# oso95/Agentainer-lab

Measured on AMD Instinct MI355X. Metric: concurrent_agent_chat_req_per_s, higher is better.
Workload: dtype bf16; 1 GPU; model=llama3-8b, agents_per_gpu=64, agents=64, global_batch=64, prompt_len=256, gen_len=57, seq_len=313, parallelism=dp1

## Files before the change

### agentainer_amd/ops/csrc/decode_attn.hip

```cpp

#include <torch/extension.h>
#include <ATen/hip/HIPContext.h>
#include <cfloat>
#include "common.h"

namespace {

constexpr int CHUNK = 64;
constexpr int SPLITS = 8;
constexpr int PART_STRIDE = 132;

template <int RATIO, int D, typename CT>
__global__ __launch_bounds__(64) void decode_partial_kernel(
    float* __restrict__ part,
    const short* __restrict__ q,
    const CT* __restrict__ k_cache,
    const CT* __restrict__ v_cache,
    const int* __restrict__ page_table,
    const int* __restrict__ seq_lens,
    float scale, int n_q, int n_kv, int PS, int max_pages, long q_ts) {
  constexpr bool FP8 = sizeof(CT) == 1;
  const int b = blockIdx.x;
  const int g = blockIdx.y;
  const int split = blockIdx.z;
  const int lane = threadIdx.x;
  const int len = seq_lens[b];
  constexpr int D8 = D / 8;

  float* my_part = part +
      ((((long)b * gridDim.y + g) * SPLITS + split) * RATIO) * PART_STRIDE;

  const int n_chunks = (len + CHUNK - 1) / CHUNK;
  const int cpw = (n_chunks + SPLITS - 1) / SPLITS;
  const int c0 = split * cpw;
  const int c1 = min(c0 + cpw, n_chunks);
  if (len <= 0 || c0 >= c1) {
    for (int h = 0; h < RATIO; ++h) {
      float* pp = my_part + h * PART_STRIDE;
      pp[2 * lane] = 0.f;
      pp[2 * lane + 1] = 0.f;
      if (lane == 0) { pp[128] = -FLT_MAX; pp[129] = 0.f; }
    }
    return;
  }

  __shared__ float p_lds[RATIO][CHUNK];
  const int qh0 = g * RATIO;
  const int ds = lane / 16;
  const int t16 = lane % 16;
  typedef __bf16 bf2 __attribute__((ext_vector_type(2)));
  __shared__ short q_lds[RATIO][D];
#pragma unroll
  for (int h = 0; h < RATIO; ++h) {
    const short* qp = q + (long)b * q_ts + (long)(qh0 + h) * D;
#pragma unroll
    for (int r = 0; r < D / WAVE; ++r)
      q_lds[h][r * WAVE + lane] = qp[r * WAVE + lane];
  }
  __builtin_amdgcn_s_waitcnt(0);

  constexpr int Q8S = D + 8;
  __shared__ unsigned char q8_lds[16 * Q8S];
  __shared__ float qsc_lds[16];
  if constexpr (sizeof(CT) == 1) {
#pragma unroll
    for (int h = 0; h < 16; ++h) {
      float sc = 0.f;
      if (h < RATIO) {
        float mx = fmaxf(fabsf(bits2f(q_lds[h][2 * lane])),
                         fabsf(bits2f(q_lds[h][2 * lane + 1])));
        mx = wave_max(mx);
        sc = fmaxf(mx, 1e-8f) / 448.f;
        const float inv = 1.f / sc;
        q8_lds[h * Q8S + 2 * lane] =
            f2fp8(bits2f(q_lds[h][2 * lane]) * inv);
        q8_lds[h * Q8S + 2 * lane + 1] =
            f2fp8(bits2f(q_lds[h][2 * lane + 1]) * inv);
      } else {
        q8_lds[h * Q8S + 2 * lane] = 0;
        q8_lds[h * Q8S + 2 * lane + 1] = 0;
      }
      if (lane == 0) qsc_lds[h] = sc;
    }
    __builtin_amdgcn_s_waitcnt(0);
  }

  const int pv_tg = lane / 16;
  const int pv_dg = lane % 16;
  float m[RATIO], l[RATIO];
  float o[RATIO][8];
#pragma unroll
  for (int h = 0; h < RATIO; ++h) {
    m[h] = -FLT_MAX; l[h] = 0.f;
#pragma unroll
    for (int j = 0; j < 8; ++j) o[h][j] = 0.f;
  }
  const int* pt = page_table + (long)b * max_pages;

  for (int c = c0; c < c1; ++c) {
    if constexpr (FP8) {
      __shared__ float cm_b[16], cs_b[16], mn_b[16];
      const int myh = lane % 16;
      float sv[16];
#pragma unroll
      for (int gt = 0; gt < 4; ++gt) {
        const int tok = c * CHUNK + gt * 16 + (lane % 16);
        const int tok_c = min(tok, len - 1);
        const long page = pt[tok_c / PS];
        const CT* kp = k_cache +
            ((long)page * n_kv + g) * D8 * PS * 8 + (tok_c % PS) * 8;
        f32x4 acc = {0.f, 0.f, 0.f, 0.f};
#pragma unroll
        for (int dc = 0; dc < 4; ++dc) {
          long a, bq;
          __builtin_memcpy(&a, kp + (long)(dc * 4 + lane / 16) * PS * 8, 8);
          __builtin_memcpy(&bq, &q8_lds[myh * Q8S + dc * 32 + (lane / 16) * 8],
                           8);
          acc = __builtin_amdgcn_mfma_f32_16x16x32_fp8_fp8(a, bq, acc, 0, 0, 0);
        }
#pragma unroll
        for (int r = 0; r < 4; ++r) sv[gt * 4 + r] = acc[r];
      }
      const float qs = qsc_lds[myh] * scale;
      float cmax = -FLT_MAX;
#pragma unroll
      for (int gt = 0; gt < 4; ++gt)
#pragma unroll
        for (int r = 0; r < 4; ++r) {
          const int tok = c * CHUNK + gt * 16 + (lane / 16) * 4 + r;
          const float v = (tok < len) ? sv[gt * 4 + r] * qs : -FLT_MAX;
          sv[gt * 4 + r] = v;
          cmax = fmaxf(cmax, v);
        }
      cmax = fmaxf(cmax, __shfl_xor(cmax, 16, WAVE));
      cmax = fmaxf(cmax, __shfl_xor(cmax, 32, WAVE));
      if (lane < 16) cm_b[myh] = cmax;
      __builtin_amdgcn_s_waitcnt(0);
      float alpha_s[RATIO];
#pragma unroll
      for (int h = 0; h < RATIO; ++h) {
        const float mn = fmaxf(m[h], cm_b[h]);
        alpha_s[h] = (m[h] == -FLT_MAX) ? 0.f : __expf(m[h] - mn);
#pragma unroll
        for (int j = 0; j < 8; ++j) o[h][j] *= alpha_s[h];
        m[h] = mn;
        if (lane == 0) mn_b[h] = mn;
      }
      __builtin_amdgcn_s_waitcnt(0);
      const float mn_my = mn_b[myh];
      float csum = 0.f;
#pragma unroll
      for (int gt = 0; gt < 4; ++gt)
#pragma unroll
        for (int r = 0; r < 4; ++r) {
          const int t = gt * 16 + (lane / 16) * 4 + r;
          const float pv = (sv[gt * 4 + r] == -FLT_MAX)
                               ? 0.f
                               : __expf(sv[gt * 4 + r] - mn_my);
          if (myh < RATIO) p_lds[myh][t] = pv;
          csum += pv;
        }
      csum += __shfl_xor(csum, 16, WAVE);
      csum += __shfl_xor(csum, 32, WAVE);
      if (lane < 16) cs_b[myh] = csum;
      __builtin_amdgcn_s_waitcnt(0);
#pragma unroll
      for (int h = 0; h < RATIO; ++h) l[h] = l[h] * alpha_s[h] + cs_b[h];
    } else {
    float s[4][RATIO];
#pragma unroll
    for (int sub = 0; sub < 4; ++sub) {
      const int tok = c * CHUNK + sub * 16 + t16;
      float acc[RATIO];
#pragma unroll
      for (int h = 0; h < RATIO; ++h) acc[h] = 0.f;
      if (tok < len) {
        const long page = pt[tok / PS];
        const CT* kp = k_cache +
            ((long)page * n_kv + g) * D8 * PS * 8 + (tok % PS) * 8;
        {
          bf16x8 kv[4];
#pragma unroll
          for (int r = 0; r < 4; ++r)
            kv[r] = *reinterpret_cast<const bf16x8*>(
                kp + (long)(r * 4 + ds) * PS * 8);
#pragma unroll
          for (int r = 0; r < 4; ++r) {
            const bf2* kp2 = reinterpret_cast<const bf2*>(&kv[r]);
#pragma unroll
            for (int h = 0; h < RATIO; ++h) {
              const bf16x8 qv8 = *reinterpret_cast<const bf16x8*>(
                  &q_lds[h][(r * 4 + ds) * 8]);
              const bf2* qp2 = reinterpret_cast<const bf2*>(&qv8);
#pragma unroll
              for (int j = 0; j < 4; ++j)
                acc[h] = __builtin_amdgcn_fdot2_f32_bf16(kp2[j], qp2[j],
                                                         acc[h], false);
            }
          }
        }
      }
#pragma unroll
      for (int h = 0; h < RATIO; ++h) {
        acc[h] += __shfl_xor(acc[h], 16, WAVE);
        acc[h] += __shfl_xor(acc[h], 32, WAVE);
        s[sub][h] = (tok < len) ? acc[h] * scale : -FLT_MAX;
      }
    }
#pragma unroll
    for (int h = 0; h < RATIO; ++h) {
      float cm = fmaxf(fmaxf(s[0][h], s[1][h]), fmaxf(s[2][h], s[3][h]));
      cm = wave_max(cm);
      const float mn = fmaxf(m[h], cm);
      float psum = 0.f;
#pragma unroll
      for (int sub = 0; sub < 4; ++sub) {
        const float p = (s[sub][h] == -FLT_MAX) ? 0.f : __expf(s[sub][h] - mn);
        if (ds == 0) {
          p_lds[h][sub * 16 + t16] = p;
          psum += p;
        }
      }
      const float csum = wave_sum(psum);
      const float alpha = (m[h] == -FLT_MAX) ? 0.f : __expf(m[h] - mn);
      l[h] = l[h] * alpha + csum;
#pragma unroll
      for (int j = 0; j < 8; ++j) o[h][j] *= alpha;
      m[h] = mn;
    }
    __builtin_amdgcn_s_waitcnt(0);
    }

    const int base_tok = c * CHUNK;
#pragma unroll 4
    for (int u = 0; u < 16; ++u) {
      const int t = u * 4 + pv_tg;
      const int gt = base_tok + t;
      const int gt_c = min(gt, len - 1);
      const long page = pt[gt_c / PS];
      const CT* vp = v_cache +
          (((long)page * n_kv + g) * PS + gt_c % PS) * D + pv_dg * 8;
      float vf[8];
      if constexpr (FP8) {
        const u8x8 vv = *reinterpret_cast<const u8x8*>(vp);
        fp8x8_to_f32(vv, vf);
      } else {
        const bf16x8 vv = *reinterpret_cast<const bf16x8*>(vp);
#pragma unroll
        for (int j = 0; j < 8; ++j) vf[j] = bits2f(vv[j]);
      }
#pragma unroll
      for (int h = 0; h < RATIO; ++h) {
        const float pw = p_lds[h][t];
#pragma unroll
        for (int j = 0; j < 8; ++j)
          o[h][j] = fmaf(pw, vf[j], o[h][j]);
      }
    }
  }

#pragma unroll
  for (int h = 0; h < RATIO; ++h) {
    float* pp = my_part + h * PART_STRIDE;
#pragma unroll
    for (int j = 0; j < 8; ++j) {
      float v = o[h][j];
      v += __shfl_xor(v, 16, WAVE);
      v += __shfl_xor(v, 32, WAVE);
      if (pv_tg == 0) pp[pv_dg * 8 + j] = v;
    }
    if (lane == 0) { pp[128] = m[h]; pp[129] = l[h]; }
  }
}

template <int D>
__global__ __launch_bounds__(64) void decode_combine_kernel(
    short* __restrict__ out,
    const float* __restrict__ part,
    const int* __restrict__ seq_lens, int n_q, int n_kv) {
  const int b = blockIdx.x;
  const int qh = blockIdx.y;
  const int lane = threadIdx.x;
  if (seq_lens[b] <= 0) return;
  const int ratio = n_q / n_kv;
  const int g = qh / ratio;
  const int h = qh % ratio;
  const float* pp = part +
      ((((long)b * n_kv + g) * SPLITS) * ratio + h) * PART_STRIDE;
  const long step = (long)ratio * PART_STRIDE;

  float M = -FLT_MAX;
#pragma unroll
  for (int s = 0; s < SPLITS; ++s) M = fmaxf(M, pp[s * step + 128]);
  float L = 0.f, O0 = 0.f, O1 = 0.f;
#pragma unroll
  for (int s = 0; s < SPLITS; ++s) {
    const float ms = pp[s * step + 128];
    if (ms == -FLT_MAX) continue;
    const float w = __expf(ms - M);
    L += w * pp[s * step + 129];
    O0 = fmaf(w, pp[s * step + 2 * lane], O0);
    O1 = fmaf(w, pp[s * step + 2 * lane + 1], O1);
  }
  const float inv = (L > 0.f) ? 1.0f / L : 0.f;
  short* op = out + ((long)b * n_q + qh) * D + 2 * lane;
  op[0] = f2bits(O0 * inv);
  op[1] = f2bits(O1 * inv);
}

}

void paged_decode_attention_ws(torch::Tensor out, torch::Tensor q,
                               torch::Tensor k_cache, torch::Tensor v_cache,
                               torch::Tensor page_table, torch::Tensor seq_lens,
                               torch::Tensor workspace, double scale) {
  TORCH_CHECK(out.is_contiguous());
  TORCH_CHECK(q.scalar_type() == at::kBFloat16);
  TORCH_CHECK(page_table.scalar_type() == at::kInt &&
              seq_lens.scalar_type() == at::kInt);
  TORCH_CHECK(workspace.scalar_type() == at::kFloat);
  TORCH_CHECK(q.stride(2) == 1 && q.stride(1) == q.size(2));
  const int B = q.size(0), n_q = q.size(1), D = q.size(2);
  const int n_kv = k_cache.size(1), PS = k_cache.size(3);
  const int max_pages = page_table.size(1);
  const int ratio = n_q / n_kv;
  TORCH_CHECK(D == 128, "decode attention: head_dim 128 only");
  TORCH_CHECK(n_q % n_kv == 0);
  TORCH_CHECK(workspace.numel() >=
              (long)B * n_kv * SPLITS * ratio * PART_STRIDE,
              "decode workspace too small");
  if (B == 0) return;
  auto stream = at::hip::getCurrentHIPStream();
  dim3 grid1(B, n_kv, SPLITS);
  const bool fp8 = k_cache.scalar_type() == at::kFloat8_e4m3fn;
#define LAUNCH_RATIO_CT(R, CT)                                                 \
  hipLaunchKernelGGL((decode_partial_kernel<R, 128, CT>), grid1, dim3(64), 0,  \
                     stream, workspace.data_ptr<float>(),                      \
                     (const short*)q.data_ptr(),                               \
                     (const CT*)k_cache.data_ptr(),                            \
                     (const CT*)v_cache.data_ptr(),                            \
                     page_table.data_ptr<int>(), seq_lens.data_ptr<int>(),     \
                     (float)scale, n_q, n_kv, PS, max_pages,                    \
                     (long)q.stride(0))
#define LAUNCH_RATIO(R)                                                        \
  do {                                                                         \
    if (fp8) LAUNCH_RATIO_CT(R, unsigned char);                                \
    else LAUNCH_RATIO_CT(R, short);                                            \
  } while (0)
  switch (ratio) {
    case 1: LAUNCH_RATIO(1); break;
    case 2: LAUNCH_RATIO(2); break;
    case 4: LAUNCH_RATIO(4); break;
    case 8: LAUNCH_RATIO(8); break;
    default:
      TORCH_CHECK(false, "decode attention: GQA ratio must be 1/2/4/8, got ",
                  ratio);
  }
#undef LAUNCH_RATIO
#undef LAUNCH_RATIO_CT
  hipLaunchKernelGGL((decode_combine_kernel<128>), dim3(B, n_q), dim3(64), 0,
                     stream, (short*)out.data_ptr(),
                     workspace.data_ptr<float>(), seq_lens.data_ptr<int>(),
                     n_q, n_kv);
}

long decode_attention_workspace_size(long B, long n_q, long n_kv) {
  return B * n_kv * SPLITS * (n_q / n_kv) * PART_STRIDE;
}

void paged_decode_attention(torch::Tensor out, torch::Tensor q,
                            torch::Tensor k_cache, torch::Tensor v_cache,
                            torch::Tensor page_table, torch::Tensor seq_lens,
                            double scale) {
  const int B = q.size(0), n_q = q.size(1);
  const int n_kv = k_cache.size(1);
  auto ws = torch::empty(
      {decode_attention_workspace_size(B, n_q, n_kv)},
      torch::TensorOptions().dtype(torch::kFloat).device(q.device()));
  paged_decode_attention_ws(out, q, k_cache, v_cache, page_table, seq_lens,
                            ws, scale);
}
```

Baseline: 126.0 req/s.

## Fuse split-K decode attention and combine into one multi-wave block kernel

Replaces the two-kernel split-K decode attention (partial kernel over a SPLITS grid dimension, then a combine kernel through a global workspace) with a single kernel. Each block runs SPLITS waves, the partial results are merged in LDS, and the workspace round trip and second launch go away. For power-of-two page sizes it also adds a FAST path: page ids are prefetched one chunk ahead with readfirstlane and shift/mask addressing, K loads for a whole chunk are batched, and V uses a sliding prefetch window. Full waitcnt(0) calls are relaxed to LDS-only waits. The trade-offs are fewer blocks (B*n_kv instead of B*n_kv*SPLITS), higher register pressure from the buffered loads, and removal of the workspace-based API entry points that other code may still call.

```diff
diff --git a/agentainer_amd/ops/csrc/decode_attn.hip b/agentainer_amd/ops/csrc/decode_attn.hip
--- a/agentainer_amd/ops/csrc/decode_attn.hip
+++ b/agentainer_amd/ops/csrc/decode_attn.hip
@@ -10,61 +10,68 @@
 constexpr int SPLITS = 8;
 constexpr int PART_STRIDE = 132;
 
-template <int RATIO, int D, typename CT>
-__global__ __launch_bounds__(64) void decode_partial_kernel(
-    float* __restrict__ part,
+template <int D>
+__device__ __forceinline__ void merge_partials(short* __restrict__ op,
+                                               const float* pp, int step,
+                                               int lane) {
+  float M = -FLT_MAX;
+#pragma unroll
+  for (int s = 0; s < SPLITS; ++s) M = fmaxf(M, pp[s * step + 128]);
+  float L = 0.f, O0 = 0.f, O1 = 0.f;
+#pragma unroll
+  for (int s = 0; s < SPLITS; ++s) {
+    const float ms = pp[s * step + 128];
+    if (ms == -FLT_MAX) continue;
+    const float w = __expf(ms - M);
+    L += w * pp[s * step + 129];
+    O0 = fmaf(w, pp[s * step + 2 * lane], O0);
+    O1 = fmaf(w, pp[s * step + 2 * lane + 1], O1);
+  }
+  const float inv = (L > 0.f) ? 1.0f / L : 0.f;
+  op[0] = f2bits(O0 * inv);
+  op[1] = f2bits(O1 * inv);
+}
+
+template <int RATIO, int D, typename CT, bool FAST>
+__global__ __launch_bounds__(SPLITS * WAVE) void decode_attn_kernel(
+    short* __restrict__ out,
     const short* __restrict__ q,
     const CT* __restrict__ k_cache,
     const CT* __restrict__ v_cache,
     const int* __restrict__ page_table,
     const int* __restrict__ seq_lens,
-    float scale, int n_q, int n_kv, int PS, int max_pages, long q_ts) {
+    float scale, int n_q, int n_kv, int PS, int ps_shift, int max_pages,
+    long q_ts) {
   constexpr bool FP8 = sizeof(CT) == 1;
+  constexpr int D8 = D / 8;
+  constexpr int VWIN = 8;
   const int b = blockIdx.x;
   const int g = blockIdx.y;
-  const int split = blockIdx.z;
-  const int lane = threadIdx.x;
+  const int split = __builtin_amdgcn_readfirstlane(threadIdx.x / WAVE);
+  const int lane = threadIdx.x % WAVE;
   const int len = seq_lens[b];
-  constexpr int D8 = D / 8;
-
-  float* my_part = part +
-      ((((long)b * gridDim.y + g) * SPLITS + split) * RATIO) * PART_STRIDE;
-
-  const int n_chunks = (len + CHUNK - 1) / CHUNK;
-  const int cpw = (n_chunks + SPLITS - 1) / SPLITS;
-  const int c0 = split * cpw;
-  const int c1 = min(c0 + cpw, n_chunks);
-  if (len <= 0 || c0 >= c1) {
-    for (int h = 0; h < RATIO; ++h) {
-      float* pp = my_part + h * PART_STRIDE;
-      pp[2 * lane] = 0.f;
-      pp[2 * lane + 1] = 0.f;
-      if (lane == 0) { pp[128] = -FLT_MAX; pp[129] = 0.f; }
-    }
-    return;
-  }
-
-  __shared__ float p_lds[RATIO][CHUNK];
+  if (len <= 0) return;
+
+  __shared__ float part_lds[SPLITS][RATIO][PART_STRIDE];
+  __shared__ float p_all[SPLITS][RATIO][CHUNK];
+  float (*p_lds)[CHUNK] = p_all[split];
   const int qh0 = g * RATIO;
   const int ds = lane / 16;
   const int t16 = lane % 16;
   typedef __bf16 bf2 __attribute__((ext_vector_type(2)));
   __shared__ short q_lds[RATIO][D];
-#pragma unroll
-  for (int h = 0; h < RATIO; ++h) {
-    const short* qp = q + (long)b * q_ts + (long)(qh0 + h) * D;
-#pragma unroll
-    for (int r = 0; r < D / WAVE; ++r)
-      q_lds[h][r * WAVE + lane] = qp[r * WAVE + lane];
-  }
-  __builtin_amdgcn_s_waitcnt(0);
+  for (int i = threadIdx.x; i < RATIO * D; i += SPLITS * WAVE)
+    q_lds[i / D][i % D] = q[(long)b * q_ts + (long)(qh0 + i / D) * D + i % D];
+  __syncthreads();
 
   constexpr int Q8S = D + 8;
-  __shared__ unsigned char q8_lds[16 * Q8S];
+  __shared__ unsigned char q8_lds[FP8 ? 16 * Q8S : 1];
   __shared__ float qsc_lds[16];
-  if constexpr (sizeof(CT) == 1) {
-#pragma unroll
-    for (int h = 0; h < 16; ++h) {
+  __shared__ float cm_all[SPLITS][16], cs_all[SPLITS][16], mn_all[SPLITS][16];
+  if constexpr (FP8) {
+#pragma unroll
+    for (int hh = 0; hh < 16 / SPLITS; ++hh) {
+      const int h = split + hh * SPLITS;
       float sc = 0.f;
       if (h < RATIO) {
         float mx = fmaxf(fabsf(bits2f(q_lds[h][2 * lane])),
@@ -82,7 +89,7 @@
       }
       if (lane == 0) qsc_lds[h] = sc;
     }
-    __builtin_amdgcn_s_waitcnt(0);
+    __syncthreads();
   }
 
   const int pv_tg = lane / 16;
@@ -96,30 +103,99 @@
     for (int j = 0; j < 8; ++j) o[h][j] = 0.f;
   }
   const int* pt = page_table + (long)b * max_pages;
+  const int psm = PS - 1;
+
+  const int n_chunks = (len + CHUNK - 1) / CHUNK;
+  const int cpw = (n_chunks + SPLITS - 1) / SPLITS;
+  const int c0 = split * cpw;
+  const int c1 = min(c0 + cpw, n_chunks);
+
+  int pid_n[4] = {0, 0, 0, 0};
+  if constexpr (FAST) {
+    if (c0 < c1) {
+#pragma unroll
+      for (int j = 0; j < 4; ++j)
+        pid_n[j] = __builtin_amdgcn_readfirstlane(
+            pt[min(c0 * CHUNK + j * 16, len - 1) >> ps_shift]);
+    }
+  }
+
+  using VT = typename std::conditional<FP8, u8x8, bf16x8>::type;
 
   for (int c = c0; c < c1; ++c) {
+    int pid[4];
+#pragma unroll
+    for (int j = 0; j < 4; ++j) pid[j] = pid_n[j];
+    if constexpr (FAST) {
+#pragma unroll
+      for (int j = 0; j < 4; ++j)
+        pid_n[j] = __builtin_amdgcn_readfirstlane(
+            pt[min((c + 1) * CHUNK + j * 16, len - 1) >> ps_shift]);
+    }
+    const int base_tok = c * CHUNK;
+    auto k_ptr = [&](int j, int tok_c, int d8) -> const CT* {
+      if constexpr (FAST) {
+        const char* base = reinterpret_cast<const char*>(
+            k_cache + ((long)pid[j] * n_kv + g) * D8 * PS * 8);
+        const unsigned boff =
+            (unsigned)((d8 * PS + (tok_c & psm)) * 8) * (unsigned)sizeof(CT);
+        return reinterpret_cast<const CT*>(base + boff);
+      } else {
+        const long page = pt[tok_c / PS];
+        return k_cache + ((long)page * n_kv + g) * D8 * PS * 8 +
+               (tok_c % PS) * 8 + (long)d8 * PS * 8;
+      }
+    };
+    auto v_ptr = [&](int u) -> const CT* {
+      const int gt_c = min(base_tok + u * 4 + pv_tg, len - 1);
+      if constexpr (FAST) {
+        const char* base = reinterpret_cast<const char*>(
+            v_cache + ((long)pid[u / 4] * n_kv + g) * PS * D);
+        const unsigned boff =
+            (unsigned)((gt_c & psm) * D + pv_dg * 8) * (unsigned)sizeof(CT);
+        return reinterpret_cast<const CT*>(base + boff);
+      } else {
+        const long page = pt[gt_c / PS];
+        return v_cache + (((long)page * n_kv + g) * PS + gt_c % PS) * D +
+               pv_dg * 8;
+      }
+    };
+    VT vb[16];
+    constexpr int KA = FAST ? 4 : 1;
+
     if constexpr (FP8) {
-      __shared__ float cm_b[16], cs_b[16], mn_b[16];
+      float* cm_b = cm_all[split];
+      float* cs_b = cs_all[split];
+      float* mn_b = mn_all[split];
       const int myh = lane % 16;
       float sv[16];
 #pragma unroll
-      for (int gt = 0; gt < 4; ++gt) {
-        const int tok = c * CHUNK + gt * 16 + (lane % 16);
-        const int tok_c = min(tok, len - 1);
-        const long page = pt[tok_c / PS];
-        const CT* kp = k_cache +
-            ((long)page * n_kv + g) * D8 * PS * 8 + (tok_c % PS) * 8;
-        f32x4 acc = {0.f, 0.f, 0.f, 0.f};
-#pragma unroll
-        for (int dc = 0; dc < 4; ++dc) {
-          long a, bq;
-          __builtin_memcpy(&a, kp + (long)(dc * 4 + lane / 16) * PS * 8, 8);
-          __builtin_memcpy(&bq, &q8_lds[myh * Q8S + dc * 32 + (lane / 16) * 8],
-                           8);
-          acc = __builtin_amdgcn_mfma_f32_16x16x32_fp8_fp8(a, bq, acc, 0, 0, 0);
-        }
-#pragma unroll
-        for (int r = 0; r < 4; ++r) sv[gt * 4 + r] = acc[r];
+      for (int g0 = 0; g0 < 4; g0 += KA) {
+        long ka[KA][4];
+#pragma unroll
+        for (int a = 0; a < KA; ++a) {
+          const int tok = c * CHUNK + (g0 + a) * 16 + (lane % 16);
+          const int tok_c = min(tok, len - 1);
+#pragma unroll
+          for (int dc = 0; dc < 4; ++dc)
+            __builtin_memcpy(&ka[a][dc],
+                             k_ptr(g0 + a, tok_c, dc * 4 + lane / 16), 8);
+        }
+#pragma unroll
+        for (int a = 0; a < KA; ++a) {
+          const int gt = g0 + a;
+          f32x4 acc = {0.f, 0.f, 0.f, 0.f};
+#pragma unroll
+          for (int dc = 0; dc < 4; ++dc) {
+            long bq;
+            __builtin_memcpy(
+                &bq, &q8_lds[myh * Q8S + dc * 32 + (lane / 16) * 8], 8);
+            acc = __builtin_amdgcn_mfma_f32_16x16x32_fp8_fp8(ka[a][dc], bq,
+                                                             acc, 0, 0, 0);
+          }
+#pragma unroll
+          for (int r = 0; r < 4; ++r) sv[gt * 4 + r] = acc[r];
+        }
       }
       const float qs = qsc_lds[myh] * scale;
       float cmax = -FLT_MAX;
@@ -135,7 +211,7 @@
       cmax = fmaxf(cmax, __shfl_xor(cmax, 16, WAVE));
       cmax = fmaxf(cmax, __shfl_xor(cmax, 32, WAVE));
       if (lane < 16) cm_b[myh] = cmax;
-      __builtin_amdgcn_s_waitcnt(0);
+      __builtin_amdgcn_s_waitcnt(0xC07F);
       float alpha_s[RATIO];
 #pragma unroll
       for (int h = 0; h < RATIO; ++h) {
@@ -146,7 +222,7 @@
         m[h] = mn;
         if (lane == 0) mn_b[h] = mn;
       }
-      __builtin_amdgcn_s_waitcnt(0);
+      __builtin_amdgcn_s_waitcnt(0xC07F);
       const float mn_my = mn_b[myh];
       float csum = 0.f;
 #pragma unroll
@@ -163,41 +239,42 @@
       csum += __shfl_xor(csum, 16, WAVE);
       csum += __shfl_xor(csum, 32, WAVE);
       if (lane < 16) cs_b[myh] = csum;
-      __builtin_amdgcn_s_waitcnt(0);
+      __builtin_amdgcn_s_waitcnt(0xC07F);
 #pragma unroll
       for (int h = 0; h < RATIO; ++h) l[h] = l[h] * alpha_s[h] + cs_b[h];
     } else {
     float s[4][RATIO];
 #pragma unroll
-    for (int sub = 0; sub < 4; ++sub) {
+    for (int s0 = 0; s0 < 4; s0 += KA) {
+      bf16x8 kv[KA][4];
+#pragma unroll
+      for (int a = 0; a < KA; ++a) {
+        const int tok_c = min(c * CHUNK + (s0 + a) * 16 + t16, len - 1);
+#pragma unroll
+        for (int r = 0; r < 4; ++r)
+          kv[a][r] = *reinterpret_cast<const bf16x8*>(
+              k_ptr(s0 + a, tok_c, r * 4 + ds));
+      }
+#pragma unroll
+      for (int a = 0; a < KA; ++a) {
+      const int sub = s0 + a;
       const int tok = c * CHUNK + sub * 16 + t16;
+      asm volatile("" ::: "memory");
       float acc[RATIO];
 #pragma unroll
       for (int h = 0; h < RATIO; ++h) acc[h] = 0.f;
-      if (tok < len) {
-        const long page = pt[tok / PS];
-        const CT* kp = k_cache +
-            ((long)page * n_kv + g) * D8 * PS * 8 + (tok % PS) * 8;
-        {
-          bf16x8 kv[4];
-#pragma unroll
-          for (int r = 0; r < 4; ++r)
-            kv[r] = *reinterpret_cast<const bf16x8*>(
-                kp + (long)(r * 4 + ds) * PS * 8);
-#pragma unroll
-          for (int r = 0; r < 4; ++r) {
-            const bf2* kp2 = reinterpret_cast<const bf2*>(&kv[r]);
-#pragma unroll
-            for (int h = 0; h < RATIO; ++h) {
-              const bf16x8 qv8 = *reinterpret_cast<const bf16x8*>(
-                  &q_lds[h][(r * 4 + ds) * 8]);
-              const bf2* qp2 = reinterpret_cast<const bf2*>(&qv8);
-#pragma unroll
-              for (int j = 0; j < 4; ++j)
-                acc[h] = __builtin_amdgcn_fdot2_f32_bf16(kp2[j], qp2[j],
-                                                         acc[h], false);
-            }
-          }
+#pragma unroll
+      for (int r = 0; r < 4; ++r) {
+        const bf2* kp2 = reinterpret_cast<const bf2*>(&kv[a][r]);
+#pragma unroll
+        for (int h = 0; h < RATIO; ++h) {
+          const bf16x8 qv8 = *reinterpret_cast<const bf16x8*>(
+              &q_lds[h][(r * 4 + ds) * 8]);
+          const bf2* qp2 = reinterpret_cast<const bf2*>(&qv8);
+#pragma unroll
+          for (int j = 0; j < 4; ++j)
+            acc[h] = __builtin_amdgcn_fdot2_f32_bf16(kp2[j], qp2[j],
+                                                     acc[h], false);
         }
       }
 #pragma unroll
@@ -205,6 +282,7 @@
         acc[h] += __shfl_xor(acc[h], 16, WAVE);
         acc[h] += __shfl_xor(acc[h], 32, WAVE);
         s[sub][h] = (tok < len) ? acc[h] * scale : -FLT_MAX;
+      }
       }
     }
 #pragma unroll
@@ -228,24 +306,15 @@
       for (int j = 0; j < 8; ++j) o[h][j] *= alpha;
       m[h] = mn;
     }
-    __builtin_amdgcn_s_waitcnt(0);
-    }
-
-    const int base_tok = c * CHUNK;
-#pragma unroll 4
-    for (int u = 0; u < 16; ++u) {
+    __builtin_amdgcn_s_waitcnt(0xC07F);
+    }
+
+    auto pv_step = [&](int u, const VT vv) {
       const int t = u * 4 + pv_tg;
-      const int gt = base_tok + t;
-      const int gt_c = min(gt, len - 1);
-      const long page = pt[gt_c / PS];
-      const CT* vp = v_cache +
-          (((long)page * n_kv + g) * PS + gt_c % PS) * D + pv_dg * 8;
       float vf[8];
       if constexpr (FP8) {
-        const u8x8 vv = *reinterpret_cast<const u8x8*>(vp);
         fp8x8_to_f32(vv, vf);
       } else {
-        const bf16x8 vv = *reinterpret_cast<const bf16x8*>(vp);
 #pragma unroll
         for (int j = 0; j < 8; ++j) vf[j] = bits2f(vv[j]);
       }
@@ -256,12 +325,31 @@
         for (int j = 0; j < 8; ++j)
           o[h][j] = fmaf(pw, vf[j], o[h][j]);
       }
+    };
+    if constexpr (FAST) {
+#pragma unroll
+      for (int u = 0; u < VWIN; ++u)
+        vb[u] = *reinterpret_cast<const VT*>(v_ptr(u));
+#pragma unroll
+      for (int grp = 0; grp < 4; ++grp) {
+        asm volatile("" ::: "memory");
+#pragma unroll
+        for (int u = grp * 4 + VWIN; u < grp * 4 + VWIN + 4; ++u)
+          if (u < 16)
+            vb[u] = *reinterpret_cast<const VT*>(v_ptr(u));
+#pragma unroll
+        for (int u = grp * 4; u < grp * 4 + 4; ++u) pv_step(u, vb[u]);
+      }
+    } else {
+#pragma unroll 4
+      for (int u = 0; u < 16; ++u)
+        pv_step(u, *reinterpret_cast<const VT*>(v_ptr(u)));
     }
   }
 
 #pragma unroll
   for (int h = 0; h < RATIO; ++h) {
-    float* pp = my_part + h * PART_STRIDE;
+    float* pp = part_lds[split][h];
 #pragma unroll
     for (int j = 0; j < 8; ++j) {
       float v = o[h][j];
@@ -271,54 +359,23 @@
     }
     if (lane == 0) { pp[128] = m[h]; pp[129] = l[h]; }
   }
+  __syncthreads();
+
+  for (int h = split; h < RATIO; h += SPLITS)
+    merge_partials<D>(out + ((long)b * n_q + qh0 + h) * D + 2 * lane,
+                      part_lds[0][h], RATIO * PART_STRIDE, lane);
 }
 
-template <int D>
-__global__ __launch_bounds__(64) void decode_combine_kernel(
-    short* __restrict__ out,
-    const float* __restrict__ part,
-    const int* __restrict__ seq_lens, int n_q, int n_kv) {
-  const int b = blockIdx.x;
-  const int qh = blockIdx.y;
-  const int lane = threadIdx.x;
-  if (seq_lens[b] <= 0) return;
-  const int ratio = n_q / n_kv;
-  const int g = qh / ratio;
-  const int h = qh % ratio;
-  const float* pp = part +
-      ((((long)b * n_kv + g) * SPLITS) * ratio + h) * PART_STRIDE;
-  const long step = (long)ratio * PART_STRIDE;
-
-  float M = -FLT_MAX;
-#pragma unroll
-  for (int s = 0; s < SPLITS; ++s) M = fmaxf(M, pp[s * step + 128]);
-  float L = 0.f, O0 = 0.f, O1 = 0.f;
-#pragma unroll
-  for (int s = 0; s < SPLITS; ++s) {
-    const float ms = pp[s * step + 128];
-    if (ms == -FLT_MAX) continue;
-    const float w = __expf(ms - M);
-    L += w * pp[s * step + 129];
-    O0 = fmaf(w, pp[s * step + 2 * lane], O0);
-    O1 = fmaf(w, pp[s * step + 2 * lane + 1], O1);
-  }
-  const float inv = (L > 0.f) ? 1.0f / L : 0.f;
-  short* op = out + ((long)b * n_q + qh) * D + 2 * lane;
-  op[0] = f2bits(O0 * inv);
-  op[1] = f2bits(O1 * inv);
 }
 
-}
-
-void paged_decode_attention_ws(torch::Tensor out, torch::Tensor q,
-                               torch::Tensor k_cache, torch::Tensor v_cache,
-                               torch::Tensor page_table, torch::Tensor seq_lens,
-                               torch::Tensor workspace, double scale) {
+void paged_decode_attention(torch::Tensor out, torch::Tensor q,
+                            torch::Tensor k_cache, torch::Tensor v_cache,
+                            torch::Tensor page_table, torch::Tensor seq_lens,
+                            double scale) {
   TORCH_CHECK(out.is_contiguous());
   TORCH_CHECK(q.scalar_type() == at::kBFloat16);
   TORCH_CHECK(page_table.scalar_type() == at::kInt &&
               seq_lens.scalar_type() == at::kInt);
-  TORCH_CHECK(workspace.scalar_type() == at::kFloat);
   TORCH_CHECK(q.stride(2) == 1 && q.stride(1) == q.size(2));
   const int B = q.size(0), n_q = q.size(1), D = q.size(2);
   const int n_kv = k_cache.size(1), PS = k_cache.size(3);
@@ -326,57 +383,41 @@
   const int ratio = n_q / n_kv;
   TORCH_CHECK(D == 128, "decode attention: head_dim 128 only");
   TORCH_CHECK(n_q % n_kv == 0);
-  TORCH_CHECK(workspace.numel() >=
-              (long)B * n_kv * SPLITS * ratio * PART_STRIDE,
-              "decode workspace too small");
   if (B == 0) return;
   auto stream = at::hip::getCurrentHIPStream();
-  dim3 grid1(B, n_kv, SPLITS);
+  dim3 grid(B, n_kv);
   const bool fp8 = k_cache.scalar_type() == at::kFloat8_e4m3fn;
-#define LAUNCH_RATIO_CT(R, CT)                                                 \
-  hipLaunchKernelGGL((decode_partial_kernel<R, 128, CT>), grid1, dim3(64), 0,  \
-                     stream, workspace.data_ptr<float>(),                      \
+  const bool fast = PS >= 16 && (PS & (PS - 1)) == 0;
+  int ps_shift = 0;
+  while ((1 << ps_shift) < PS) ++ps_shift;
+#define LAUNCH_RATIO_CT(R, CT, F)                                              \
+  hipLaunchKernelGGL((decode_attn_kernel<R, 128, CT, F>), grid,                \
+                     dim3(SPLITS * WAVE), 0, stream, (short*)out.data_ptr(),   \
                      (const short*)q.data_ptr(),                               \
                      (const CT*)k_cache.data_ptr(),                            \
                      (const CT*)v_cache.data_ptr(),                            \
                      page_table.data_ptr<int>(), seq_lens.data_ptr<int>(),     \
-                     (float)scale, n_q, n_kv, PS, max_pages,                    \
+                     (float)scale, n_q, n_kv, PS, ps_shift, max_pages,         \
                      (long)q.stride(0))
-#define LAUNCH_RATIO(R)                                                        \
+#define LAUNCH_RATIO(R, FAST_OK)                                               \
   do {                                                                         \
-    if (fp8) LAUNCH_RATIO_CT(R, unsigned char);                                \
-    else LAUNCH_RATIO_CT(R, short);                                            \
+    if (fp8) {                                                                 \
+      if (FAST_OK && fast) LAUNCH_RATIO_CT(R, unsigned char, FAST_OK);         \
+      else LAUNCH_RATIO_CT(R, unsigned char, false);                           \
+    } else {                                                                   \
+      if (FAST_OK && fast) LAUNCH_RATIO_CT(R, short, FAST_OK);                 \
+      else LAUNCH_RATIO_CT(R, short, false);                                   \
+    }                                                                          \
   } while (0)
   switch (ratio) {
-    case 1: LAUNCH_RATIO(1); break;
-    case 2: LAUNCH_RATIO(2); break;
-    case 4: LAUNCH_RATIO(4); break;
-    case 8: LAUNCH_RATIO(8); break;
+    case 1: LAUNCH_RATIO(1, true); break;
+    case 2: LAUNCH_RATIO(2, true); break;
+    case 4: LAUNCH_RATIO(4, true); break;
+    case 8: LAUNCH_RATIO(8, false); break;
     default:
       TORCH_CHECK(false, "decode attention: GQA ratio must be 1/2/4/8, got ",
                   ratio);
   }
 #undef LAUNCH_RATIO
 #undef LAUNCH_RATIO_CT
-  hipLaunchKernelGGL((decode_combine_kernel<128>), dim3(B, n_q), dim3(64), 0,
-                     stream, (short*)out.data_ptr(),
-                     workspace.data_ptr<float>(), seq_lens.data_ptr<int>(),
-                     n_q, n_kv);
 }
-
-long decode_attention_workspace_size(long B, long n_q, long n_kv) {
-  return B * n_kv * SPLITS * (n_q / n_kv) * PART_STRIDE;
-}
-
-void paged_decode_attention(torch::Tensor out, torch::Tensor q,
-                            torch::Tensor k_cache, torch::Tensor v_cache,
-                            torch::Tensor page_table, torch::Tensor seq_lens,
-                            double scale) {
-  const int B = q.size(0), n_q = q.size(1);
-  const int n_kv = k_cache.size(1);
-  auto ws = torch::empty(
-      {decode_attention_workspace_size(B, n_q, n_kv)},
-      torch::TensorOptions().dtype(torch::kFloat).device(q.device()));
-  paged_decode_attention_ws(out, q, k_cache, v_cache, page_table, seq_lens,
-                            ws, scale);
-}
```

Result: faster. 127.8 req/s (median of 6 runs) (+1.4%).
